# Tongdongq/darwin-gpu

Measured on AMD Instinct MI355X. Metric: GACT GCUPS (DP cells/s) on ~10 kb PacBio-shape reads, higher is better.
Workload: dtype int16x2 (packed); 1 GPU; ecoli10x_self_overlap; tile_size=320, tile_overlap=120, scoring=+1/-1/-1/-1, reads=4642, bases=48503677, candidates=65766, tiles=2185214, parallelism=candidates dealt round-robin over 1 GPU(s), slots_in_flight=4, passes_in_this_process=127, arch=gfx950:sramecc+:xnack-

## Files before the change

darwin-gpu_amd/csrc/gact_lin.hpp:

```cpp
#pragma once

#include "gact_p16s.hpp"

namespace gact {

#ifndef GACT_LIN_MAX3
#define GACT_LIN_MAX3 1
#endif
constexpr int kLinFloor = GACT_LIN_MAX3 ? 1024 : 0;
__host__ __device__ constexpr int lin_base(int g) { return kLinFloor + 40 * (-g) + 8; }
__device__ __forceinline__ uint32_t vconst(uint32_t s)
{
    uint32_t r;
    asm volatile("s_nop 1\n\tv_mov_b32 %0, %1" : "=v"(r) : "s"(s));
    return r;
}

__host__ inline bool p16_lin_ok(int tile, int match, int mismatch, int open, int ext)
{
    const long long steps = (long long)tile + 4 * kGroup + 64 + 48;
    return open == ext && mismatch == ext && ext <= 0 && match >= 0 &&
           p16_tagged_ok(tile, match, mismatch, open, ext) &&
           4 * ((long long)match * (tile + 2) + (long long)(-ext) * steps + kLinFloor) + 3 <= 30000 && match - ext <= 63;
}

#ifndef GACT_LIN_BUILTINS
#define GACT_LIN_BUILTINS 0
#endif
__host__ inline bool lin_col_drift_ok(int match, int ext) { return match - 2 * ext <= 63; }
constexpr bool kLinSplitBuiltins = true;
typedef short LinS2 __attribute__((ext_vector_type(2)));
template <bool BUILTIN = GACT_LIN_BUILTINS>
__device__ __forceinline__ uint32_t lin_max(uint32_t a, uint32_t b)
{
    if constexpr (BUILTIN)
        return __builtin_bit_cast(uint32_t, __builtin_elementwise_max(__builtin_bit_cast(LinS2, a), __builtin_bit_cast(LinS2, b)));
    else
        return pk_max(a, b);
}
__device__ __forceinline__ uint32_t lin_sub(uint32_t a, uint32_t b)
{
#if GACT_LIN_BUILTINS
    return __builtin_bit_cast(uint32_t, (LinS2)(__builtin_bit_cast(LinS2, a) - __builtin_bit_cast(LinS2, b)));
#else
    return pk_sub(a, b);
#endif
}
__device__ __forceinline__ uint32_t pk_mad4v(uint32_t a, uint32_t v_c)
{
    uint32_t r;
    asm("v_pk_mad_u16 %0, %1, 4, %2 op_sel_hi:[1,0,1]" : "=v"(r) : "v"(a), "v"(v_c));
    return r;
}
__device__ __forceinline__ uint32_t pk_max3f(uint32_t a, uint32_t b, uint32_t c)
{
    uint32_t r;
    asm("v_pk_maximum3_f16 %0, %1, %2, %3" : "=v"(r) : "v"(a), "v"(b), "v"(c));
    return r;
}
__device__ __forceinline__ uint32_t pk_max3f_s(uint32_t a, uint32_t s_b, uint32_t c)
{
    uint32_t r;
    asm("v_pk_maximum3_f16 %0, %1, %2, %3" : "=v"(r) : "v"(a), "s"(s_b), "v"(c));
    return r;
}
__device__ __forceinline__ uint32_t pk_max_sgpr(uint32_t a, uint32_t s_b)
{
    uint32_t r;
    asm("v_pk_max_i16 %0, %1, %2" : "=v"(r) : "v"(a), "s"(s_b));
    return r;
}
#define GACT_DPP_SHR1 " row_shr:1 row_mask:0xf bank_mask:0xf"
#define GACT_DPP_ROR1 " row_ror:1 row_mask:0xf bank_mask:0xf"
__device__ __forceinline__ uint32_t lin_hand_shr1(uint32_t h, uint32_t v_k, uint32_t s_old)
{
    uint32_t r;
    asm("v_mov_b32 %0, %3\n\ts_nop 0\n\tv_sub_u32_dpp %0, %1, %2" GACT_DPP_SHR1 : "=&v"(r) : "v"(h), "v"(v_k), "s"(s_old));
    return r;
}
__device__ __forceinline__ uint32_t lin_hand_ror1_shr1(uint32_t h1, uint32_t v_k1, uint32_t h2, uint32_t v_k2)
{
    uint32_t r;
    asm("s_nop 1\n\tv_sub_u32_dpp %0, %1, %2" GACT_DPP_ROR1 "\n\tv_sub_u32_dpp %0, %3, %4" GACT_DPP_SHR1
        : "=&v"(r) : "v"(h1), "v"(v_k1), "v"(h2), "v"(v_k2));
    return r;
}
__device__ __forceinline__ uint32_t lin_hand_scaled_ror1(uint32_t h1, uint32_t v_c)
{
    uint32_t r;
    asm("v_pk_mad_u16 %0, %1, 4, %2 op_sel_hi:[1,0,1]\n\ts_nop 1\n\tv_mov_b32_dpp %0, %0" GACT_DPP_ROR1 : "=&v"(r) : "v"(h1), "v"(v_c));
    return r;
}
__device__ __forceinline__ uint32_t lin_hand_shr1_over(uint32_t first, uint32_t h2, uint32_t v_k2)
{
    asm("s_nop 1\n\tv_sub_u32_dpp %0, %1, %2" GACT_DPP_SHR1 : "+v"(first) : "v"(h2), "v"(v_k2));
    return first;
}
template <bool BUILTIN = GACT_LIN_BUILTINS>
__device__ __forceinline__ uint32_t andn_or(uint32_t a, uint32_t b, uint32_t c)
{
    if constexpr (BUILTIN)
        return __builtin_amdgcn_bitop3_b32(a, b, c, 0xba);
    else {
        uint32_t r;
        asm("v_bitop3_b32 %0, %1, %2, %3 bitop3:0xba" : "=v"(r) : "v"(a), "v"(b), "v"(c));
        return r;
    }
}
__device__ __forceinline__ uint32_t pk_ashr2(uint32_t a)
{
#if GACT_LIN_BUILTINS
    return __builtin_bit_cast(uint32_t, (LinS2)(__builtin_bit_cast(LinS2, a) >> (short)2));
#else
    uint32_t r;
    asm("v_pk_ashrrev_i16 %0, 2, %1 op_sel_hi:[0,1]" : "=v"(r) : "v"(a));
    return r;
#endif
}


__device__ __forceinline__ uint32_t sconst_here(uint32_t lit)
{
    uint32_t r;
    asm volatile("s_mov_b32 %0, %1" : "=s"(r) : "i"(lit));
    return r;
}

template <int CW> struct LinWords {
    static constexpr int kWords = (CW + 1) / 2;
    static constexpr int kUint4 = (kWords + 3) / 4;
};
template <int NW, int LANES, class Fix>
__device__ __forceinline__ void lin_flush(const uint32_t (&acc)[2 * NW], uint4 *qA, uint4 *qB, Fix fix, const bool storeA, const bool storeB)
{
    constexpr int QD = (NW + 3) / 4;
    uint32_t wa[QD * 4], wb[QD * 4];
#pragma unroll
    for (int n = 0; n < QD * 4; n++) {
        wa[n] = n < NW ? fix(__builtin_amdgcn_perm(acc[n < NW ? 2 * n + 1 : 0], acc[n < NW ? 2 * n : 0], 0x05040100u)) : 0u;
        wb[n] = n < NW ? fix(__builtin_amdgcn_perm(acc[n < NW ? 2 * n + 1 : 0], acc[n < NW ? 2 * n : 0], 0x07060302u)) : 0u;
    }
    if (storeA) {
#pragma unroll
        for (int q = 0; q < QD; q++) qA[q * kWsRow] = make_uint4(wa[4 * q], wa[4 * q + 1], wa[4 * q + 2], wa[4 * q + 3]);
    }
    if (storeB) {
#pragma unroll
        for (int q = 0; q < QD; q++) qB[q * kWsRow] = make_uint4(wb[4 * q], wb[4 * q + 1], wb[4 * q + 2], wb[4 * q + 3]);
    }
}

template <int S> struct LinPos { static constexpr int value = S; };
constexpr int kLinTail = -1;
constexpr uint32_t kLinPairSel = 0x06020400u;
constexpr uint32_t kLinPairMask = 0x03030303u;
constexpr uint32_t kLinFlushSelA = 0x05010400u;
constexpr uint32_t kLinFlushSelB = 0x07030602u;
template <int CW>
__device__ __forceinline__ void lin_flush_groups(const uint32_t (&grp)[2 * (CW / 2)], const uint32_t odd, uint4 *qA, uint4 *qB,
                                                 const bool storeA, const bool storeB)
{
    constexpr int NP = CW / 2, NW = LinWords<CW>::kWords, QD = LinWords<CW>::kUint4;
    uint32_t wa[QD * 4], wb[QD * 4];
    const uint32_t sA = sconst_here(kLinFlushSelA), sB = sconst_here(kLinFlushSelB);
#pragma unroll
    for (int n = 0; n < QD * 4; n++) {
        wa[n] = n < NP ? __builtin_amdgcn_perm(grp[n < NP ? 2 * n : 0], grp[n < NP ? 2 * n + 1 : 0], sA)
              : n < NW ? odd & 0xffffu : 0u;
        wb[n] = n < NP ? __builtin_amdgcn_perm(grp[n < NP ? 2 * n : 0], grp[n < NP ? 2 * n + 1 : 0], sB)
              : n < NW ? odd >> 16 : 0u;
    }
    if (storeA) {
#pragma unroll
        for (int q = 0; q < QD; q++) qA[q * kWsRow] = make_uint4(wa[4 * q], wa[4 * q + 1], wa[4 * q + 2], wa[4 * q + 3]);
    }
    if (storeB) {
#pragma unroll
        for (int q = 0; q < QD; q++) qB[q * kWsRow] = make_uint4(wb[4 * q], wb[4 * q + 1], wb[4 * q + 2], wb[4 * q + 3]);
    }
}

constexpr int kLinBandDefault = 48, kLinBandMin = 24, kLinBandQuantum = 1;
struct LinBand {
    int lo[2], hi[2];
    bool full[2];
    __device__ __forceinline__ bool store(int h, int first, int last) const { return full[h] | ((last >= lo[h]) & (first <= hi[h])); }
};
__device__ __forceinline__ void lin_band_range(LinBand &b, int h, int T_end, int behind, int dj_min, int dj_max, int band, bool full)
{
    b.full[h] = full | (band <= 0);
    b.lo[h] = T_end - behind - dj_max - band;
    b.hi[h] = dj_max < 0 ? -0x40000000 : T_end - behind - imax(dj_min, 0) + band;
}

template <int C1, int C2>
__device__ __forceinline__ uint32_t dp_pass_lin_split(const P16Consts &kc, const int gl,
                                                      const uint16_t *__restrict__ ref16,
                                                      const uint32_t (&qb)[C1 + C2],
                                                      const int T_end, const int tB,
                                                      uint32_t *__restrict__ wsA, uint32_t *__restrict__ wsB,
                                                      const int band, const bool fullA, const bool fullB,
                                                      const uint32_t *lut_lds)
{
    constexpr int CT = C1 + C2;
    constexpr int NW = LinWords<C2>::kWords, QD = LinWords<C2>::kUint4;
    constexpr int LAG = kGroup;
    const int g = (int)(int16_t)(kc.ext & 0xffffu);
    const uint32_t gv = vconst(kc.next), g4v = vconst(kc.next4), c3v = vconst(kc.c3), onev = vconst(kc.one),
                   dtv = vconst(kc.next4 + kc.tag1),
                   c2v = vconst(kc.tag2);
    const uint32_t psel = sconst_here(kLinPairSel);
    uint32_t Z1 = pk2(lin_base(g) + gl * g), Z2 = pk2(lin_base(g) + (gl + LAG) * g);
    uint32_t G[CT];
    uint32_t acc[2 * NW];
    uint32_t grp[2 * (C2 / 2)], odd = 0;
#pragma unroll
    for (int c = 0; c < CT; c++) G[c] = c < C1 ? Z1 : Z2;
#pragma unroll
    for (int c = 0; c < 2 * NW; c++) acc[c] = 0;
    uint32_t H1 = Z1, H2 = Z2;
    uint32_t Hdiag1 = Z1, Hdiag2 = Z2;

    typedef __attribute__((address_space(3))) const uint8_t LdsByte;
    typedef __attribute__((address_space(3))) const uint32_t LdsWord;
    LdsByte *const lut_plain = (LdsByte *)lut_lds, *const lut_tagged = (LdsByte *)(lut_lds + 1);
    auto row = [](LdsByte *table, uint32_t stream_byte) { return *(LdsWord *)(table + stream_byte); };
    LdsByte *rp = (LdsByte *)(ref16 + (1 - LAG));
    uint32_t rb1 = row(lut_plain, rp[2 * LAG]), rb1b = row(lut_plain, rp[2 * LAG + 1]);
    uint32_t rb2 = row(lut_plain, rp[0]), rb2b = row(lut_plain, rp[1]);
    rp += 2;

#define GACT_SB() __builtin_amdgcn_sched_barrier(0)
    uint32_t sb1 = 0, sb1b = 0, sb2 = 0, sb2b = 0;
    auto ask_bytes = [&](const bool r1, const bool r2) {
        if (r2) { sb2 = rp[0]; sb2b = rp[1]; }
        if (r1) { sb1 = rp[2 * LAG]; sb1b = rp[2 * LAG + 1]; }
        rp += 2;
    };
    auto ask_rows = [&](const bool r1, const bool r2, const bool tag2) {
        if (r1) { rb1 = row(lut_plain, sb1); rb1b = row(lut_plain, sb1b); }
        if (r2) { rb2 = row(tag2 ? lut_tagged : lut_plain, sb2); rb2b = row(tag2 ? lut_tagged : lut_plain, sb2b); }
    };
    auto upper_all = [&](uint32_t (&U)[CT], const bool tag2, const uint32_t Zr2) {
        uint32_t P[CT];
#pragma unroll
        for (int c = 0; c < CT; c++) P[c] = __builtin_amdgcn_perm(c < C1 ? rb1b : rb2b, c < C1 ? rb1 : rb2, qb[c]);
        GACT_SB();
#pragma unroll
        for (int c = 0; c < CT; c++) U[c] = (c == 0 ? Hdiag1 : c == C1 ? Hdiag2 : G[c - 1]) + P[c];
        ask_rows(true, true, tag2);
        GACT_SB();
        if (GACT_LIN_MAX3) {
#pragma unroll
            for (int c = 0; c < CT; c++)
                U[c] = pk_max3f(U[c], c < C1 ? Z1 : Zr2, G[c]);
        } else {
#pragma unroll
            for (int c = 0; c < CT; c++) U[c] = lin_max(U[c], c < C1 ? Z1 : Zr2);
            GACT_SB();
#pragma unroll
            for (int c = 0; c < CT; c++) U[c] = lin_max(U[c], G[c]);
        }
        GACT_SB();
    };

    auto step = [&]() {
        ask_bytes(true, true);
        Z1 += gv; Z2 += gv;
        const uint32_t Hl1 = (uint32_t)dpp_row_shr1((int)H1, (int)Z1);
        const uint32_t Hl2 = (uint32_t)dpp_row_shr1((int)H2, dpp_row_ror1((int)H1));
        uint32_t U[CT];
        upper_all(U, false, Z2);
        Hdiag1 = Hl1; Hdiag2 = Hl2;
        uint32_t Ha = Hl1, Hb = Hl2;
        static_assert(C2 >= C1, "region 2 is the longer chain");
#pragma unroll
        for (int c = 0; c < C1; c++) {
            const uint32_t Da = Ha - gv, Db = Hb - gv;
            GACT_SB();
            G[c] = lin_max(U[c], Da); G[C1 + c] = lin_max(U[C1 + c], Db);
            GACT_SB();
            Ha = G[c]; Hb = G[C1 + c];
        }
#pragma unroll
        for (int c = 2 * C1; c < CT; c++) { G[c] = lin_max(U[c], Hb - gv); Hb = G[c]; }
        H1 = Ha; H2 = Hb;
    };
    auto step_r1 = [&]() {
        ask_bytes(true, false);
        Z1 += gv; Z2 += gv;
        const uint32_t Hl1 = (uint32_t)dpp_row_shr1((int)H1, (int)Z1);
        uint32_t P[C1], U[C1];
#pragma unroll
        for (int c = 0; c < C1; c++) P[c] = __builtin_amdgcn_perm(rb1b, rb1, qb[c]);
        GACT_SB();
#pragma unroll
        for (int c = 0; c < C1; c++) U[c] = (c == 0 ? Hdiag1 : G[c - 1]) + P[c];
        ask_rows(true, false, false);
        GACT_SB();
#pragma unroll
        for (int c = 0; c < C1; c++) U[c] = GACT_LIN_MAX3 ? pk_max3f(U[c], Z1, G[c]) : lin_max(lin_max(U[c], Z1), G[c]);
        GACT_SB();
        Hdiag1 = Hl1;
        uint32_t Ha = Hl1;
#pragma unroll
        for (int c = 0; c < C1; c++) { G[c] = lin_max(U[c], Ha - gv); Ha = G[c]; }
        H1 = Ha;
    };

    uint32_t Z24 = 0;
    static_assert(C2 >= 3 && (C2 & 1), "the last pair is filed while the unpaired slot is computed");
    auto file_group = [&](const int S, const int c, const uint32_t x) {
        uint32_t &r = grp[c - 2 + (S >> 2)];
        r = (S & 3) ? pk_shl_add4(r, x) : x;
    };
    auto step_tagged = [&](auto pos) {
        constexpr int S = decltype(pos)::value;
        constexpr bool blk = S != kLinTail;
        ask_bytes(true, true);
        Z1 += gv; Z24 += g4v;
        const uint32_t Hl1 = (uint32_t)dpp_row_shr1((int)H1, (int)Z1);
        const uint32_t Hl2 = (uint32_t)dpp_row_shr1((int)H2, dpp_row_ror1((int)pk_mad4v(H1, c2v)));
        uint32_t U[CT];
        upper_all(U, true, Z24);
        Hdiag1 = Hl1; Hdiag2 = Hl2;
        uint32_t Ha = Hl1, Hb = Hl2;
        uint32_t tprev = 0, Hq = 0, x = 0;
#pragma unroll
        for (int c = 0; c < C2; c++) {
            const bool both = c < C1;
            const bool filed = blk && c >= 2 && !(c & 1);
            uint32_t Da = 0;
            const uint32_t Db = Hb - dtv;
            if (both) Da = Ha - gv;
            if (filed) x &= kLinPairMask;
            GACT_SB();
            const uint32_t Hp = lin_max(U[C1 + c], Db);
            if (both) { G[c] = lin_max(U[c], Da); Ha = G[c]; }
            if (!blk && c > 0) acc[c - 1] = pk_shl_add4(acc[c - 1], tprev);
            if (filed) file_group(S, c, x);
            GACT_SB();
            G[C1 + c] = andn_or(Hp, c3v, c2v);
            if (!blk || c == C2 - 1) tprev = Hp & c3v;
            else if (c & 1) x = __builtin_amdgcn_perm(Hp, Hq, psel);
            else Hq = Hp;
            GACT_SB();
            Hb = G[C1 + c];
        }
        if (!blk) acc[C2 - 1] = pk_shl_add4(acc[C2 - 1], tprev);
        else odd = S ? pk_shl_add4(odd, tprev) : tprev;
        H1 = Ha; H2 = Hb;
    };
    auto step_tagged_r2 = [&](auto pos) {
        constexpr int S = decltype(pos)::value;
        constexpr bool blk = S != kLinTail;
        ask_bytes(false, true);
        Z24 += g4v;
        const uint32_t Hl2 = (uint32_t)dpp_row_shr1((int)H2, dpp_row_ror1((int)pk_mad4v(H1, c2v)));
        uint32_t P[C2], U[C2];
#pragma unroll
        for (int c = 0; c < C2; c++) P[c] = __builtin_amdgcn_perm(rb2b, rb2, qb[C1 + c]);
        GACT_SB();
#pragma unroll
        for (int c = 0; c < C2; c++) U[c] = (c == 0 ? Hdiag2 : G[C1 + c - 1]) + P[c];
        ask_rows(false, true, true);
        GACT_SB();
#pragma unroll
        for (int c = 0; c < C2; c++) U[c] = GACT_LIN_MAX3 ? pk_max3f(U[c], Z24, G[C1 + c]) : lin_max(lin_max(U[c], Z24), G[C1 + c]);
        GACT_SB();
        Hdiag2 = Hl2;
        uint32_t Hb = Hl2;
        uint32_t tprev = 0, Hq = 0, x = 0;
#pragma unroll
        for (int c = 0; c < C2; c++) {
            const bool filed = blk && c >= 2 && !(c & 1);
            const uint32_t Db = Hb - dtv;
            if (filed) x &= kLinPairMask;
            GACT_SB();
            const uint32_t Hp = lin_max(U[c], Db);
            if (!blk && c > 0) acc[c - 1] = pk_shl_add4(acc[c - 1], tprev);
            if (filed) file_group(S, c, x);
            GACT_SB();
            G[C1 + c] = andn_or(Hp, c3v, c2v);
            if (!blk || c == C2 - 1) tprev = Hp & c3v;
            else if (c & 1) x = __builtin_amdgcn_perm(Hp, Hq, psel);
            else Hq = Hp;
            GACT_SB();
            Hb = G[C1 + c];
        }
        if (!blk) acc[C2 - 1] = pk_shl_add4(acc[C2 - 1], tprev);
        else odd = S ? pk_shl_add4(odd, tprev) : tprev;
        H2 = Hb;
    };
#define GACT_LIN_BLOCK8(f) do { f(LinPos<0>{}); f(LinPos<1>{}); f(LinPos<2>{}); f(LinPos<3>{}); \
                                f(LinPos<4>{}); f(LinPos<5>{}); f(LinPos<6>{}); f(LinPos<7>{}); } while (0)
#undef GACT_SB
    auto enter_tagged = [&]() {
#pragma unroll
        for (int c = C1; c < CT; c++) G[c] = pk_mad4v(G[c], c2v);
        H2 = pk_mad4v(H2, c2v);
        Hdiag2 = pk_mad4v(Hdiag2, c2v);
        Z24 = pk_mad4v(Z2, c3v);
        rb2 = row(lut_tagged, rp[-2]); rb2b = row(lut_tagged, rp[-1]);
    };

    int t = 1;
    for (const int tP = imin(LAG, imin(tB - 1, T_end)); t <= tP; t++) step_r1();
    if (t > 1) {
#pragma unroll
        for (int c = C1; c < CT; c++) G[c] = Z2;
        H2 = Z2; Hdiag2 = Z2;
        rb2 = row(lut_plain, rp[-2]); rb2b = row(lut_plain, rp[-1]);
    }
    const int tU = imin(tB - 1, T_end);
    for (; t + 1 <= tU; t += 2) { step(); step(); }
    if (t <= tU) { step(); t++; }
    const bool tagged = t <= T_end;
    if (tagged) enter_tagged();
    uint4 *qA = reinterpret_cast<uint4 *>(wsA) + gl;
    uint4 *qB = reinterpret_cast<uint4 *>(wsB) + gl;
    LinBand bd;
    {
        const int q1 = (band >> 16) - 1, b = band & 0xffff;
        const int u_lo = kGroup - 1 - (gl & ~q1), u_hi = kGroup - 1 - (gl | q1);
        LinBand lo_, hi_;
        lin_band_range(lo_, 0, T_end, u_lo, C2 * u_lo, C2 * u_lo + C2 - 1, b, fullA);
        lin_band_range(hi_, 0, T_end, u_hi, C2 * u_hi, C2 * u_hi + C2 - 1, b, fullA);
        bd.lo[0] = bd.lo[1] = lo_.lo[0]; bd.hi[0] = bd.hi[1] = hi_.hi[0];
        bd.full[0] = fullA | (b <= 0); bd.full[1] = fullB | (b <= 0);
    }
    int k = 0;
    while (t + 7 <= T_end && t <= T_end - LAG) {
        GACT_LIN_BLOCK8(step_tagged);
        t += 8; k += 8;
        lin_flush_groups<C2>(grp, odd, qA, qB, bd.store(0, t - 8, t - 1), bd.store(1, t - 8, t - 1));
        qA += QD * kWsRow;
        qB += QD * kWsRow;
    }
    while (t + 7 <= T_end) {
        GACT_LIN_BLOCK8(step_tagged_r2);
        t += 8; k += 8;
        lin_flush_groups<C2>(grp, odd, qA, qB, bd.store(0, t - 8, t - 1), bd.store(1, t - 8, t - 1));
        qA += QD * kWsRow;
        qB += QD * kWsRow;
    }
#undef GACT_LIN_BLOCK8
    for (; t <= T_end - LAG; t++, k++) step_tagged(LinPos<kLinTail>{});
    for (; t <= T_end; t++, k++) step_tagged_r2(LinPos<kLinTail>{});
    if (k & 7) {
        const int sh = 2 * (8 - (k & 7));
        lin_flush<NW, kGroup>(acc, qA, qB, [sh](uint32_t w) { return ((w & 0xffffu) << sh & 0xffffu) | ((w >> 16) << sh << 16); },
                              bd.store(0, t - (k & 7), t - 1), bd.store(1, t - (k & 7), t - 1));
    }
    return tagged ? pk_ashr2(lin_sub(H2 | kc.c3, Z24)) : lin_sub(H2, Z2);
}

template <int C1, int C2>
__device__ __forceinline__ uint32_t dp_pass_lin_split_col(const P16Consts &kc, const int gl,
                                                      const uint16_t *__restrict__ ref16,
                                                      const uint32_t (&qb)[C1 + C2],
                                                      const int T_end, const int tB,
                                                      uint32_t *__restrict__ wsA, uint32_t *__restrict__ wsB,
                                                      const int band, const bool fullA, const bool fullB,
                                                      const uint32_t *lut_lds)
{
    constexpr int CT = C1 + C2;
    constexpr int NW = LinWords<C2>::kWords, QD = LinWords<C2>::kUint4;
    constexpr int LAG = kGroup;
    const int g = (int)(int16_t)(kc.ext & 0xffffu);
    const uint32_t gs = kc.next, g4s = kc.next4;
    const uint32_t k1v = vconst((uint32_t)(C1 - 1) * kc.next),
                   k2v = vconst((uint32_t)(C2 - 1) * kc.next);
    uint32_t c3v = 0, onev = 0, c2v = 0,
             k24v = 0,
             k12v = 0;
    const uint32_t psel = sconst_here(kLinPairSel);
    constexpr int NWIN = C2 + 1;
    uint32_t W[NWIN], T[C2];
#pragma unroll
    for (int k = 0; k < NWIN; k++) W[k] = pk2(lin_base(g) + (k - 1) * (-g));
#pragma unroll
    for (int c = 0; c < C2; c++) T[c] = 0;
    auto bump = [](uint32_t &z, const uint32_t by) { asm("s_add_u32 %0, %0, %1" : "+s"(z) : "s"(by) : "scc"); };
    auto advance = [&](const int nW, const bool tagged_too) {
#pragma unroll
        for (int k = 0; k < NWIN; k++) if (k < nW) { if (tagged_too) bump(W[k], gs); else W[k] += gs; }
        if (tagged_too) {
#pragma unroll
            for (int c = 0; c < C2; c++) bump(T[c], g4s);
        }
    };
    uint32_t G[CT];
    uint32_t acc[2 * NW];
    uint32_t grp[2 * (C2 / 2)], odd = 0;
#pragma unroll
    for (int c = 0; c < CT; c++) G[c] = W[(c < C1 ? c : c - C1) + 1];
#pragma unroll
    for (int c = 0; c < 2 * NW; c++) acc[c] = 0;
    uint32_t H1 = W[C1], H2 = W[C2];
    uint32_t Hdiag1 = W[0], Hdiag2 = W[0];

    typedef __attribute__((address_space(3))) const uint8_t LdsByte;
    typedef __attribute__((address_space(3))) const uint32_t LdsWord;
    LdsByte *const lut_plain = (LdsByte *)lut_lds, *const lut_tagged = (LdsByte *)(lut_lds + 1);
    auto row = [](LdsByte *table, uint32_t stream_byte) { return *(LdsWord *)(table + stream_byte); };
    LdsByte *rp = (LdsByte *)(ref16 + (1 - LAG));
    uint32_t rb1 = row(lut_plain, rp[2 * LAG]), rb1b = row(lut_plain, rp[2 * LAG + 1]);
    uint32_t rb2 = row(lut_plain, rp[0]), rb2b = row(lut_plain, rp[1]);
    rp += 2;

#define GACT_SB() __builtin_amdgcn_sched_barrier(0)
    uint32_t sb1 = 0, sb1b = 0, sb2 = 0, sb2b = 0;
    auto ask_bytes = [&](const bool r1, const bool r2) {
        if (r2) { sb2 = rp[0]; sb2b = rp[1]; }
        if (r1) { sb1 = rp[2 * LAG]; sb1b = rp[2 * LAG + 1]; }
        rp += 2;
    };
    auto ask_rows = [&](const bool r1, const bool r2, const bool tag2) {
        if (r1) { rb1 = row(lut_plain, sb1); rb1b = row(lut_plain, sb1b); }
        if (r2) { rb2 = row(tag2 ? lut_tagged : lut_plain, sb2); rb2b = row(tag2 ? lut_tagged : lut_plain, sb2b); }
    };
    auto upper_all = [&](uint32_t (&U)[CT], const bool tag2) {
        uint32_t P[CT];
#pragma unroll
        for (int c = 0; c < CT; c++) P[c] = __builtin_amdgcn_perm(c < C1 ? rb1b : rb2b, c < C1 ? rb1 : rb2, qb[c]);
        GACT_SB();
#pragma unroll
        for (int c = 0; c < CT; c++) U[c] = (c == 0 ? Hdiag1 : c == C1 ? Hdiag2 : G[c - 1]) + P[c];
        ask_rows(true, true, tag2);
        GACT_SB();
        if (GACT_LIN_MAX3) {
#pragma unroll
            for (int c = 0; c < CT; c++)
                U[c] = pk_max3f_s(U[c], c < C1 ? W[c + 1] : tag2 ? T[c - C1] : W[c - C1 + 1], G[c]);
        } else {
#pragma unroll
            for (int c = 0; c < CT; c++) U[c] = pk_max_sgpr(U[c], c < C1 ? W[c + 1] : tag2 ? T[c - C1] : W[c - C1 + 1]);
            GACT_SB();
#pragma unroll
            for (int c = 0; c < CT; c++) U[c] = lin_max<kLinSplitBuiltins>(U[c], G[c]);
        }
        GACT_SB();
    };

    auto step = [&]() {
        ask_bytes(true, true);
        advance(NWIN, false);
        const uint32_t Hl1 = lin_hand_shr1(H1, k1v, W[0]);
        const uint32_t Hl2 = lin_hand_ror1_shr1(H1, k1v, H2, k2v);
        uint32_t U[CT];
        upper_all(U, false);
        Hdiag1 = Hl1; Hdiag2 = Hl2;
        uint32_t Ha = Hl1, Hb = Hl2;
        static_assert(C2 >= C1, "region 2 is the longer chain");
#pragma unroll
        for (int c = 0; c < C1; c++) {
            G[c] = lin_max<kLinSplitBuiltins>(U[c], Ha); G[C1 + c] = lin_max<kLinSplitBuiltins>(U[C1 + c], Hb);
            GACT_SB();
            Ha = G[c]; Hb = G[C1 + c];
        }
#pragma unroll
        for (int c = 2 * C1; c < CT; c++) { G[c] = lin_max<kLinSplitBuiltins>(U[c], Hb); Hb = G[c]; }
        H1 = Ha; H2 = Hb;
    };
    auto step_r1 = [&]() {
        ask_bytes(true, false);
        advance(C1 + 1, false);
        const uint32_t Hl1 = lin_hand_shr1(H1, k1v, W[0]);
        uint32_t P[C1], U[C1];
#pragma unroll
        for (int c = 0; c < C1; c++) P[c] = __builtin_amdgcn_perm(rb1b, rb1, qb[c]);
        GACT_SB();
#pragma unroll
        for (int c = 0; c < C1; c++) U[c] = (c == 0 ? Hdiag1 : G[c - 1]) + P[c];
        ask_rows(true, false, false);
        GACT_SB();
#pragma unroll
        for (int c = 0; c < C1; c++) U[c] = GACT_LIN_MAX3 ? pk_max3f_s(U[c], W[c + 1], G[c]) : lin_max<kLinSplitBuiltins>(pk_max_sgpr(U[c], W[c + 1]), G[c]);
        GACT_SB();
        Hdiag1 = Hl1;
        uint32_t Ha = Hl1;
#pragma unroll
        for (int c = 0; c < C1; c++) { G[c] = lin_max<kLinSplitBuiltins>(U[c], Ha); Ha = G[c]; }
        H1 = Ha;
    };

    static_assert(C2 >= 3 && (C2 & 1), "the last pair is filed while the unpaired slot is computed");
    auto file_group = [&](const int S, const int c, const uint32_t x) {
        uint32_t &r = grp[c - 2 + (S >> 2)];
        r = (S & 3) ? pk_shl_add4(r, x) : x;
    };
    auto step_tagged = [&](auto pos) {
        constexpr int S = decltype(pos)::value;
        constexpr bool blk = S != kLinTail;
        ask_bytes(true, true);
        advance(C1 + 1, true);
        const uint32_t Hl1 = lin_hand_shr1(H1, k1v, W[0]);
        const uint32_t Hl2 = lin_hand_shr1_over(lin_hand_scaled_ror1(H1, k12v), H2, k24v);
        uint32_t U[CT];
        upper_all(U, true);
        Hdiag1 = Hl1; Hdiag2 = Hl2;
        uint32_t Ha = Hl1, Hb = Hl2;
        uint32_t tprev = 0, Hq = 0, x = 0;
#pragma unroll
        for (int c = 0; c < C2; c++) {
            const bool both = c < C1;
            const bool filed = blk && c >= 2 && !(c & 1);
            const uint32_t Db = Hb - onev;
            if (filed) x &= kLinPairMask;
            GACT_SB();
            const uint32_t Hp = lin_max<kLinSplitBuiltins>(U[C1 + c], Db);
            if (both) { G[c] = lin_max<kLinSplitBuiltins>(U[c], Ha); Ha = G[c]; }
            if (!blk && c > 0) acc[c - 1] = pk_shl_add4(acc[c - 1], tprev);
            if (filed) file_group(S, c, x);
            GACT_SB();
            G[C1 + c] = andn_or<kLinSplitBuiltins>(Hp, c3v, c2v);
            if (!blk || c == C2 - 1) tprev = Hp & c3v;
            else if (c & 1) x = __builtin_amdgcn_perm(Hp, Hq, psel);
            else Hq = Hp;
            GACT_SB();
            Hb = G[C1 + c];
        }
        if (!blk) acc[C2 - 1] = pk_shl_add4(acc[C2 - 1], tprev);
        else odd = S ? pk_shl_add4(odd, tprev) : tprev;
        H1 = Ha; H2 = Hb;
    };
    auto step_tagged_r2 = [&](auto pos) {
        constexpr int S = decltype(pos)::value;
        constexpr bool blk = S != kLinTail;
        ask_bytes(false, true);
        advance(0, true);
        const uint32_t Hl2 = lin_hand_shr1_over(lin_hand_scaled_ror1(H1, k12v), H2, k24v);
        uint32_t P[C2], U[C2];
#pragma unroll
        for (int c = 0; c < C2; c++) P[c] = __builtin_amdgcn_perm(rb2b, rb2, qb[C1 + c]);
        GACT_SB();
#pragma unroll
        for (int c = 0; c < C2; c++) U[c] = (c == 0 ? Hdiag2 : G[C1 + c - 1]) + P[c];
        ask_rows(false, true, true);
        GACT_SB();
#pragma unroll
        for (int c = 0; c < C2; c++) U[c] = GACT_LIN_MAX3 ? pk_max3f_s(U[c], T[c], G[C1 + c]) : lin_max<kLinSplitBuiltins>(pk_max_sgpr(U[c], T[c]), G[C1 + c]);
        GACT_SB();
        Hdiag2 = Hl2;
        uint32_t Hb = Hl2;
        uint32_t tprev = 0, Hq = 0, x = 0;
#pragma unroll
        for (int c = 0; c < C2; c++) {
            const bool filed = blk && c >= 2 && !(c & 1);
            const uint32_t Db = Hb - onev;
            if (filed) x &= kLinPairMask;
            GACT_SB();
            const uint32_t Hp = lin_max<kLinSplitBuiltins>(U[c], Db);
            if (!blk && c > 0) acc[c - 1] = pk_shl_add4(acc[c - 1], tprev);
            if (filed) file_group(S, c, x);
            GACT_SB();
            G[C1 + c] = andn_or<kLinSplitBuiltins>(Hp, c3v, c2v);
            if (!blk || c == C2 - 1) tprev = Hp & c3v;
            else if (c & 1) x = __builtin_amdgcn_perm(Hp, Hq, psel);
            else Hq = Hp;
            GACT_SB();
            Hb = G[C1 + c];
        }
        if (!blk) acc[C2 - 1] = pk_shl_add4(acc[C2 - 1], tprev);
        else odd = S ? pk_shl_add4(odd, tprev) : tprev;
        H2 = Hb;
    };
#define GACT_LIN_BLOCK8(f) do { f(LinPos<0>{}); f(LinPos<1>{}); f(LinPos<2>{}); f(LinPos<3>{}); \
                                f(LinPos<4>{}); f(LinPos<5>{}); f(LinPos<6>{}); f(LinPos<7>{}); } while (0)
#undef GACT_SB
    auto enter_tagged = [&]() {
        c3v = vconst(kc.c3); onev = vconst(kc.one); c2v = vconst(kc.tag2);
        k24v = vconst((uint32_t)(C2 - 1) * kc.next4);
        k12v = vconst(pk2(2 + 4 * (C1 - 1) * g));
#pragma unroll
        for (int c = C1; c < CT; c++) G[c] = pk_mad4v(G[c], c2v);
        H2 = pk_mad4v(H2, c2v);
        Hdiag2 = pk_mad4v(Hdiag2, c2v);
#pragma unroll
        for (int c = 0; c < C2; c++) T[c] = (W[c + 1] << 2) + kc.c3;
        rb2 = row(lut_tagged, rp[-2]); rb2b = row(lut_tagged, rp[-1]);
    };

    int t = 1;
    for (const int tP = imin(LAG, imin(tB - 1, T_end)); t <= tP; t++) step_r1();
    if (t > 1) {
#pragma unroll
        for (int k = C1 + 1; k < NWIN; k++) W[k] = W[k - 1] + gs;
#pragma unroll
        for (int c = C1; c < CT; c++) G[c] = W[c - C1 + 1];
        H2 = W[C2]; Hdiag2 = W[0];
        rb2 = row(lut_plain, rp[-2]); rb2b = row(lut_plain, rp[-1]);
    }
    const int tU = imin(tB - 1, T_end);
    for (; t + 1 <= tU; t += 2) { step(); step(); }
    if (t <= tU) { step(); t++; }
    const bool tagged = t <= T_end;
    if (tagged) enter_tagged();
    uint4 *qA = reinterpret_cast<uint4 *>(wsA) + gl;
    uint4 *qB = reinterpret_cast<uint4 *>(wsB) + gl;
    LinBand bd;
    {
        const int q1 = (band >> 16) - 1, b = band & 0xffff;
        const int u_lo = kGroup - 1 - (gl & ~q1), u_hi = kGroup - 1 - (gl | q1);
        LinBand lo_, hi_;
        lin_band_range(lo_, 0, T_end, u_lo, C2 * u_lo, C2 * u_lo + C2 - 1, b, fullA);
        lin_band_range(hi_, 0, T_end, u_hi, C2 * u_hi, C2 * u_hi + C2 - 1, b, fullA);
        bd.lo[0] = bd.lo[1] = lo_.lo[0]; bd.hi[0] = bd.hi[1] = hi_.hi[0];
        bd.full[0] = fullA | (b <= 0); bd.full[1] = fullB | (b <= 0);
    }
    int k = 0;
    while (t + 7 <= T_end && t <= T_end - LAG) {
        GACT_LIN_BLOCK8(step_tagged);
        t += 8; k += 8;
        lin_flush_groups<C2>(grp, odd, qA, qB, bd.store(0, t - 8, t - 1), bd.store(1, t - 8, t - 1));
        qA += QD * kWsRow;
        qB += QD * kWsRow;
    }
    while (t + 7 <= T_end) {
        GACT_LIN_BLOCK8(step_tagged_r2);
        t += 8; k += 8;
        lin_flush_groups<C2>(grp, odd, qA, qB, bd.store(0, t - 8, t - 1), bd.store(1, t - 8, t - 1));
        qA += QD * kWsRow;
        qB += QD * kWsRow;
    }
#undef GACT_LIN_BLOCK8
    for (; t <= T_end - LAG; t++, k++) step_tagged(LinPos<kLinTail>{});
    for (; t <= T_end; t++, k++) step_tagged_r2(LinPos<kLinTail>{});
    if (k & 7) {
        const int sh = 2 * (8 - (k & 7));
        lin_flush<NW, kGroup>(acc, qA, qB, [sh](uint32_t w) { return ((w & 0xffffu) << sh & 0xffffu) | ((w >> 16) << sh << 16); },
                              bd.store(0, t - (k & 7), t - 1), bd.store(1, t - (k & 7), t - 1));
    }
    return tagged ? pk_ashr2(lin_sub(H2 | kc.c3, T[C2 - 1])) : lin_sub(H2, W[C2]);
}
#undef GACT_DPP_SHR1
#undef GACT_DPP_ROR1

template <int C, int LANES, bool AMAX>
__device__ __forceinline__ uint32_t dp_pass_lin(const P16Consts &kc, const int gl,
                                                const uint16_t *__restrict__ ref16,
                                                const uint32_t (&qb)[C],
                                                const int T_end, const int tB,
                                                uint32_t *__restrict__ wsA, uint32_t *__restrict__ wsB,
                                                const int cqA, const int cqB, const int (*RQ)[2], P16Best *pb,
                                                const int col_from, const int band, const int QA, const int QB,
                                                const bool fullA, const bool fullB)
{
    constexpr int NW = LinWords<C>::kWords, QD = LinWords<C>::kUint4;
    const bool store = AMAX || gl * C + C >= col_from;
    LinBand bd;
    {
        const int q1 = AMAX ? 0 : (band >> 16) - 1, b = AMAX ? 0 : band & 0xffff;
        const int g_lo = gl & ~q1, g_hi = gl | q1;
        LinBand lo_, hi_;
        lin_band_range(lo_, 0, T_end, (imax(QA, 1) - 1) / C - g_lo, QA - g_lo * C - C, QA - g_lo * C - 1, b, fullA);
        lin_band_range(lo_, 1, T_end, (imax(QB, 1) - 1) / C - g_lo, QB - g_lo * C - C, QB - g_lo * C - 1, b, fullB);
        lin_band_range(hi_, 0, T_end, (imax(QA, 1) - 1) / C - g_hi, QA - g_hi * C - C, QA - g_hi * C - 1, b, fullA);
        lin_band_range(hi_, 1, T_end, (imax(QB, 1) - 1) / C - g_hi, QB - g_hi * C - C, QB - g_hi * C - 1, b, fullB);
        bd = lo_;
        bd.hi[0] = hi_.hi[0] < 0 ? (lo_.hi[0] < 0 ? lo_.hi[0] : T_end) : hi_.hi[0];
        bd.hi[1] = hi_.hi[1] < 0 ? (lo_.hi[1] < 0 ? lo_.hi[1] : T_end) : hi_.hi[1];
    }
    static_assert(!AMAX || LANES == kGroup, "first tiles run on the 16-lane layout");
    const int g = (int)(int16_t)(kc.ext & 0xffffu);
    const uint32_t gv = vconst(kc.next), g4v = vconst(kc.next4), c3v = vconst(kc.c3), onev = vconst(kc.one),
                   dtv = vconst(kc.next4 + kc.tag1),
                   c2v = vconst(kc.tag2), lut1v = vconst(0x01010101u);
    uint32_t Z = pk2(lin_base(g) + gl * g);
    uint32_t G[C];
    uint32_t acc[2 * NW];
#pragma unroll
    for (int c = 0; c < C; c++) G[c] = Z;
#pragma unroll
    for (int c = 0; c < 2 * NW; c++) acc[c] = 0;
    uint32_t G_last = Z, Hdiag = Z;

    uint32_t bk[AMAX ? C : 1];
    int lane_best[2] = {-1, -1};
    uint32_t col_x0 = 0;
    int t_first = 0, rows[2] = {0, 0};
    if (AMAX) {
#pragma unroll
        for (int c = 0; c < C; c++) bk[c] = 0xffffffffu;
        const int ncA = imin(imax(RQ[0][1] - gl * C, 0), C), ncB = imin(imax(RQ[1][1] - gl * C, 0), C);
        col_x0 = ((uint32_t)(-ncA) & 0xffffu) | ((uint32_t)(-ncB) << 16);
        t_first = gl + 1;
        rows[0] = RQ[0][0]; rows[1] = RQ[1][0];
    }

    auto lut = [&](uint32_t amount) { return kc.dsub >> (amount & 31u); };
    auto lut4 = [&](uint32_t amount) { return kc.dsub4 >> (amount & 31u); };
    uint32_t lutA = 0, lutB = 0;
    { const uint32_t w = ref16[1]; lutA = lut(w & 0xffu); lutB = lut(w >> 8); }

    auto shr1 = [](uint32_t v, uint32_t old) {
        return (uint32_t)(LANES == 32 ? dpp_shr1_32((int)v, (int)old) : dpp_row_shr1((int)v, (int)old));
    };

#define GACT_SB() __builtin_amdgcn_sched_barrier(0)
    auto upper_all = [&](uint32_t (&U)[C], const bool tag2, const uint32_t Zr) {
        uint32_t P[C];
#pragma unroll
        for (int c = 0; c < C; c++) P[c] = __builtin_amdgcn_perm(lutB, lutA, qb[c]);
        GACT_SB();
#pragma unroll
        for (int c = 0; c < C; c++) U[c] = (c == 0 ? Hdiag : G[c - 1]) + P[c];
        (void)tag2;
        GACT_SB();
        if (GACT_LIN_MAX3) {
#pragma unroll
            for (int c = 0; c < C; c++) U[c] = pk_max3f(U[c], Zr, G[c]);
        } else {
#pragma unroll
            for (int c = 0; c < C; c++) U[c] = lin_max(U[c], Zr);
            GACT_SB();
#pragma unroll
            for (int c = 0; c < C; c++) U[c] = lin_max(U[c], G[c]);
        }
        GACT_SB();
    };

    auto step = [&](const int t) {
        const uint32_t w_next = ref16[t + 1];
        Z += gv;
        const uint32_t Hl0 = shr1(G_last, Z);
        uint32_t U[C];
        upper_all(U, false, Z);
        Hdiag = Hl0;
        uint32_t Hl = Hl0;
#pragma unroll
        for (int c = 0; c < C; c++) { G[c] = lin_max(U[c], Hl - gv); Hl = G[c]; }
        G_last = Hl;
        lutA = lut(w_next & 0xffu); lutB = lut(w_next >> 8);
    };

    uint32_t Z4 = 0, Z8 = 0;
    auto step_tagged = [&](const int t) {
        const uint32_t w_next = ref16[t + 1];
        Z4 += g4v;
        uint32_t key_c = 0;
        if (AMAX) {
            Z8 += g4v + g4v;
            const uint32_t sidx = (uint32_t)(t - tB) & 7u, row0 = (uint32_t)(t - t_first);
            const uint32_t ka = row0 < (uint32_t)rows[0] ? sidx : ((uint32_t)kKeyBias & 0xffffu);
            const uint32_t kb = row0 < (uint32_t)rows[1] ? sidx : ((uint32_t)kKeyBias & 0xffffu);
            key_c = lin_sub(ka | (kb << 16), Z8);
        }
        const uint32_t Hl0 = shr1(G_last, Z4 - onev);
        uint32_t U[C];
        upper_all(U, true, Z4);
        Hdiag = Hl0;
        uint32_t Hl = Hl0, tprev = 0;
#pragma unroll
        for (int c = 0; c < C; c++) {
            const uint32_t Db = Hl - dtv;
            GACT_SB();
            const uint32_t Hp = lin_max(U[c], Db);
            if (c > 0) {
                acc[c - 1] = pk_shl_add4(acc[c - 1], tprev);
                if (AMAX) bk[c - 1] = lin_max(bk[c - 1], pk_mad_vvv(G[c - 1], kc.tag2, key_c));
            }
            GACT_SB();
            G[c] = andn_or(Hp, c3v, c2v);
            tprev = Hp & c3v;
            GACT_SB();
            Hl = G[c];
        }
        acc[C - 1] = pk_shl_add4(acc[C - 1], tprev);
        if (AMAX) bk[C - 1] = lin_max(bk[C - 1], pk_mad_vvv(G[C - 1], kc.tag2, key_c));
        G_last = Hl;
        lutA = lut4(w_next & 0xffu) + lut1v; lutB = lut4(w_next >> 8) + lut1v;
    };
#undef GACT_SB
    auto enter_tagged = [&]() {
#pragma unroll
        for (int c = 0; c < C; c++) G[c] = pk_mad4v(G[c], c2v);
        G_last = pk_mad4v(G_last, c2v);
        Hdiag = pk_mad4v(Hdiag, c2v);
        Z4 = pk_mad4v(Z, c3v);
        Z8 = Z4 + Z4 - c2v;
        lutA = (lutA << 2) + lut1v; lutB = (lutB << 2) + lut1v;
    };

    auto fold = [&](const int kblk) {
        uint32_t m = 0xffffffffu, rel = 0, x = col_x0;
#pragma unroll
        for (int c = 0; c < C; c++) {
            const uint32_t v = pk_sign(x);
            x = pk_add(x, kc.one);
            const uint32_t key = pk_mad_m1(v, pk_add(bk[AMAX ? c : 0], kc.one));
            const uint32_t keep = pk_sign(lin_sub(key, m));
            rel = pk_mad_m1(keep, rel);
            m = lin_max(m, key);
            bk[AMAX ? c : 0] = 0xffffffffu;
        }
#pragma unroll
        for (int h = 0; h < 2; h++) {
            const int m16 = (int)(m << (16 - 16 * h)) >> 16;
            const int col = ((int)(rel << (16 - 16 * h)) >> 16) + C;
            const int rec = ((m16 >> 3) << 15) | ((kblk + (m16 & 7)) << 5) | col;
            lane_best[h] = imax(lane_best[h], m16 < 0 ? -1 : rec);
        }
    };

    int t = 1;
    for (; t < tB && t <= T_end; t++) step(t);
    const bool tagged = t <= T_end;
    if (tagged) enter_tagged();
    uint4 *qA = reinterpret_cast<uint4 *>(wsA) + gl;
    uint4 *qB = reinterpret_cast<uint4 *>(wsB) + gl;
    int k = 0;
    while (t + 7 <= T_end) {
        for (int s8 = 0; s8 < 8; s8++, t++) step_tagged(t);
        k += 8;
        lin_flush<NW, LANES>(acc, qA, qB, [](uint32_t w) { return w; }, store && bd.store(0, t - 8, t - 1), store && bd.store(1, t - 8, t - 1));
        qA += QD * kWsRow;
        qB += QD * kWsRow;
        if (AMAX) fold(k - 8);
    }
    for (; t <= T_end; t++, k++) step_tagged(t);
    if (AMAX) {
        if (k & 7) fold(k & ~7);
#pragma unroll
        for (int h = 0; h < 2; h++) {
            const int rec = lane_best[h];
            int best = 0, bi = 0, bj = 0;
            if (rec >= 0) {
                best = rec >> 15;
                bi = tB + ((rec >> 5) & 1023) - gl;
                bj = gl * C + (rec & 31) + 1;
            }
#pragma unroll
            for (int mm = 1; mm < kGroup; mm <<= 1) {
                const int ob = __shfl_xor(best, mm, kGroup);
                const int oi = __shfl_xor(bi, mm, kGroup);
                const int oj = __shfl_xor(bj, mm, kGroup);
                const bool take = (ob > best) | ((ob == best) & ((oi > bi) | ((oi == bi) & (oj > bj))));
                best = take ? ob : best;
                bi = take ? oi : bi;
                bj = take ? oj : bj;
            }
            pb->best[h] = best; pb->bi[h] = bi; pb->bj[h] = bj;
        }
    }
    if (k & 7) {
        const int sh = 2 * (8 - (k & 7));
        lin_flush<NW, LANES>(acc, qA, qB, [sh](uint32_t w) { return ((w & 0xffffu) << sh & 0xffffu) | ((w >> 16) << sh << 16); },
                             store && bd.store(0, t - (k & 7), t - 1), store && bd.store(1, t - (k & 7), t - 1));
    }
    if (AMAX) return 0;
    uint32_t ga = G[0], gb = G[0];
#pragma unroll
    for (int c = 1; c < C; c++) { ga = (c == cqA) ? G[c] : ga; gb = (c == cqB) ? G[c] : gb; }
    const uint32_t pick = __builtin_amdgcn_perm(gb, ga, 0x07060100u);
    return tagged ? pk_ashr2(lin_sub(pick | kc.c3, Z4)) : lin_sub(pick, Z);
}

struct WideLayoutLin : UniformLayout<10, 32, true> {
    static constexpr int kWalkFmt = 3, kWalkQuads = LinWords<10>::kUint4;
#ifndef GACT_WALK_SPAN
#define GACT_WALK_SPAN 16
#endif
    static constexpr int kWalkSpan = GACT_WALK_SPAN;
#ifndef GACT_WIDE_LIN_BLOCKS
#define GACT_WIDE_LIN_BLOCKS 3
#endif
    static constexpr int kBlocksPerCu = GACT_WIDE_LIN_BLOCKS;
    static constexpr bool kEndAligned = true;
    template <bool RAW>
    __device__ static uint32_t pass(const P16Consts &kc, int gl, const uint16_t *ref16, const uint32_t (&qb)[10], int T_end,
                                    int tB, uint32_t *wsA, uint32_t *wsB, const PairTile &pt)
    {
        static_assert(!RAW, "the linear-gap pass reads 2-bit sets");
        return dp_pass_lin<10, 32, false>(kc, gl, ref16, qb, T_end, tB, wsA, wsB, (imax(pt.Q[0], 1) - 1) % 10,
                                          (imax(pt.Q[1], 1) - 1) % 10, nullptr, nullptr, pt.col_from, pt.band, pt.Q[0], pt.Q[1],
                                          pt.full[0], pt.full[1]);
    }
    __device__ static int fin_lane(int Q) { return (imax(Q, 1) - 1) / 10; }
};

#ifndef GACT_LIN_BLOCKS_PER_CU
#define GACT_LIN_BLOCKS_PER_CU 3
#endif
template <int C1, int C2> struct SplitLayoutLin : SplitLayout<C1, C2, true> {
    static constexpr int kBlocksPerCu = GACT_LIN_BLOCKS_PER_CU;
    static constexpr int kWalkFmt = 3, kWalkQuads = LinWords<C2>::kUint4;
    static constexpr int kWalkSpan = GACT_WALK_SPAN;
    static constexpr bool kEndAligned = true;
    static constexpr int kLutWords = kLinLutWords;
    static constexpr bool kColDrift = true;
    using Base = SplitLayout<C1, C2, true>;
    template <bool RAW>
    __device__ static void load(const SeqSetDev &rs, const SeqSetDev &qf, const SeqSetDev &qr,
                                const PairTile &pt, int gl, uint8_t *ref8, uint8_t *q8, uint32_t (&qb)[C1 + C2], uint32_t *stage)
    {
        static_assert(!RAW, "the linear-gap pass reads 2-bit sets");
        load_pair_packed<C1 + C2, kGroup, typename Base::Cols, true, kLinPadRow>(rs, qf, qr, pt, gl, ref8, Base::G::kRefBytes, Base::G::kRow0, q8,
                                                                                 Base::G::kTileMax, qb, stage, typename Base::Cols{});
    }
    template <bool RAW>
    __device__ static uint32_t pass(const P16Consts &kc, int gl, const uint16_t *ref16, const uint32_t (&qb)[C1 + C2],
                                    int T_end, int tB, uint32_t *wsA, uint32_t *wsB, const PairTile &pt)
    {
        static_assert(!RAW, "the linear-gap pass reads 2-bit sets");
        return dp_pass_lin_split_col<C1, C2>(kc, gl, ref16, qb, T_end, tB, wsA, wsB, pt.band, pt.full[0], pt.full[1], pt.lut);
    }
    __device__ static int fin_lane(int Q) { (void)Q; return kGroup - 1; }
};

template <int C1, int C2> struct SplitLayoutLinRow : SplitLayoutLin<C1, C2> {
    static constexpr bool kColDrift = false;
    template <bool RAW>
    __device__ static uint32_t pass(const P16Consts &kc, int gl, const uint16_t *ref16, const uint32_t (&qb)[C1 + C2],
                                    int T_end, int tB, uint32_t *wsA, uint32_t *wsB, const PairTile &pt)
    {
        static_assert(!RAW, "the linear-gap pass reads 2-bit sets");
        return dp_pass_lin_split<C1, C2>(kc, gl, ref16, qb, T_end, tB, wsA, wsB, pt.band, pt.full[0], pt.full[1], pt.lut);
    }
};

template <int C1, int C2> struct SplitLayoutLinRowTeam : SplitLayoutLinRow<C1, C2> {
    static constexpr bool kTeamWalk = true;
};

template <int C1, int C2> struct SplitLayoutLinTeam : SplitLayoutLin<C1, C2> {
    static constexpr bool kTeamWalk = true;
};

}
```

Before: 9363 GCUPS.

## Slide precomputed boundary-offset strips instead of bumping scalars every step

The per-step scalar advance of the boundary arrays W and T is replaced inside 8-step blocks by precomputed strips that hold each step's offsets in extra SGPRs. Each step indexes the strip at its block position, and the whole strip is bumped once per block with batched s_add instructions. This removes the per-step SALU adds from the inner DP loop. In exchange it uses about 7 more SGPRs per array, which could affect register pressure or occupancy, and it relies on the tail loops restoring the original offsets correctly.

```diff
diff --git a/darwin-gpu_amd/csrc/gact_lin.hpp b/darwin-gpu_amd/csrc/gact_lin.hpp
--- a/darwin-gpu_amd/csrc/gact_lin.hpp
+++ b/darwin-gpu_amd/csrc/gact_lin.hpp
@@ -455,6 +455,37 @@
     return tagged ? pk_ashr2(lin_sub(H2 | kc.c3, Z24)) : lin_sub(H2, Z2);
 }
 
+#ifndef GACT_LIN_SLIDE
+#define GACT_LIN_SLIDE 1
+#endif
+constexpr int kLinBlock = 8;
+__host__ __device__ constexpr int lin_strip_len(int n, int steps = kLinBlock) { return GACT_LIN_SLIDE ? n + steps - 1 : n; }
+__host__ __device__ constexpr int lin_strip_at(int S, int k) { return GACT_LIN_SLIDE && S != kLinTail ? S + k : k; }
+template <int N, int STEPS = kLinBlock, int LEN>
+__host__ __device__ __forceinline__ void lin_strip_enter(uint32_t (&s)[LEN], const uint32_t by)
+{
+    static_assert(lin_strip_len(N, STEPS) <= LEN, "the strip fits its registers");
+#pragma unroll
+    for (int k = 0; k < N; k++) s[k] += by;
+#pragma unroll
+    for (int k = N; k < lin_strip_len(N, STEPS); k++) s[k] = s[k - 1] + by;
+}
+template <int N, int LEN>
+__host__ __device__ __forceinline__ void lin_strip_leave(uint32_t (&s)[LEN], const uint32_t by)
+{
+#pragma unroll
+    for (int k = 0; k < N; k++) s[k] -= by;
+}
+template <int N, int STEPS = kLinBlock, int LEN, class Add4, class Add1>
+__host__ __device__ __forceinline__ void lin_strip_slide(uint32_t (&s)[LEN], const uint32_t by_block, Add4 add4, Add1 add1)
+{
+    constexpr int M = lin_strip_len(N, STEPS);
+#pragma unroll
+    for (int j = 0; j + 4 <= M; j += 4) add4(s[j], s[j + 1], s[j + 2], s[j + 3], by_block);
+#pragma unroll
+    for (int j = M & ~3; j < M; j++) add1(s[j], by_block);
+}
+
 template <int C1, int C2>
 __device__ __forceinline__ uint32_t dp_pass_lin_split_col(const P16Consts &kc, const int gl,
                                                       const uint16_t *__restrict__ ref16,
@@ -476,11 +507,13 @@
              k12v = 0;
     const uint32_t psel = sconst_here(kLinPairSel);
     constexpr int NWIN = C2 + 1;
-    uint32_t W[NWIN], T[C2];
+    uint32_t W[lin_strip_len(NWIN)], T[lin_strip_len(C2)];
 #pragma unroll
     for (int k = 0; k < NWIN; k++) W[k] = pk2(lin_base(g) + (k - 1) * (-g));
 #pragma unroll
-    for (int c = 0; c < C2; c++) T[c] = 0;
+    for (int c = 0; c < lin_strip_len(C2); c++) T[c] = 0;
+#pragma unroll
+    for (int k = NWIN; k < lin_strip_len(NWIN); k++) W[k] = 0;
     auto bump = [](uint32_t &z, const uint32_t by) { asm("s_add_u32 %0, %0, %1" : "+s"(z) : "s"(by) : "scc"); };
     auto advance = [&](const int nW, const bool tagged_too) {
 #pragma unroll
@@ -489,6 +522,10 @@
 #pragma unroll
             for (int c = 0; c < C2; c++) bump(T[c], g4s);
         }
+    };
+    auto bump4 = [](uint32_t &z0, uint32_t &z1, uint32_t &z2, uint32_t &z3, const uint32_t by) {
+        asm("s_add_u32 %0, %0, %4\n\ts_add_u32 %1, %1, %4\n\ts_add_u32 %2, %2, %4\n\ts_add_u32 %3, %3, %4"
+            : "+s"(z0), "+s"(z1), "+s"(z2), "+s"(z3) : "s"(by) : "scc");
     };
     uint32_t G[CT];
     uint32_t acc[2 * NW];
@@ -520,7 +557,7 @@
         if (r1) { rb1 = row(lut_plain, sb1); rb1b = row(lut_plain, sb1b); }
         if (r2) { rb2 = row(tag2 ? lut_tagged : lut_plain, sb2); rb2b = row(tag2 ? lut_tagged : lut_plain, sb2b); }
     };
-    auto upper_all = [&](uint32_t (&U)[CT], const bool tag2) {
+    auto upper_all = [&](uint32_t (&U)[CT], const bool tag2, const int o) {
         uint32_t P[CT];
 #pragma unroll
         for (int c = 0; c < CT; c++) P[c] = __builtin_amdgcn_perm(c < C1 ? rb1b : rb2b, c < C1 ? rb1 : rb2, qb[c]);
@@ -532,10 +569,10 @@
         if (GACT_LIN_MAX3) {
 #pragma unroll
             for (int c = 0; c < CT; c++)
-                U[c] = pk_max3f_s(U[c], c < C1 ? W[c + 1] : tag2 ? T[c - C1] : W[c - C1 + 1], G[c]);
+                U[c] = pk_max3f_s(U[c], c < C1 ? W[o + c + 1] : tag2 ? T[o + c - C1] : W[o + c - C1 + 1], G[c]);
         } else {
 #pragma unroll
-            for (int c = 0; c < CT; c++) U[c] = pk_max_sgpr(U[c], c < C1 ? W[c + 1] : tag2 ? T[c - C1] : W[c - C1 + 1]);
+            for (int c = 0; c < CT; c++) U[c] = pk_max_sgpr(U[c], c < C1 ? W[o + c + 1] : tag2 ? T[o + c - C1] : W[o + c - C1 + 1]);
             GACT_SB();
 #pragma unroll
             for (int c = 0; c < CT; c++) U[c] = lin_max<kLinSplitBuiltins>(U[c], G[c]);
@@ -543,13 +580,14 @@
         GACT_SB();
     };
 
-    auto step = [&]() {
+    auto step = [&](auto pos) {
+        constexpr int S = decltype(pos)::value, o = lin_strip_at(S, 0);
         ask_bytes(true, true);
-        advance(NWIN, false);
-        const uint32_t Hl1 = lin_hand_shr1(H1, k1v, W[0]);
+        if (!GACT_LIN_SLIDE || S == kLinTail) advance(NWIN, false);
+        const uint32_t Hl1 = lin_hand_shr1(H1, k1v, W[o]);
         const uint32_t Hl2 = lin_hand_ror1_shr1(H1, k1v, H2, k2v);
         uint32_t U[CT];
-        upper_all(U, false);
+        upper_all(U, false, o);
         Hdiag1 = Hl1; Hdiag2 = Hl2;
         uint32_t Ha = Hl1, Hb = Hl2;
         static_assert(C2 >= C1, "region 2 is the longer chain");
@@ -593,12 +631,13 @@
     auto step_tagged = [&](auto pos) {
         constexpr int S = decltype(pos)::value;
         constexpr bool blk = S != kLinTail;
+        constexpr int o = lin_strip_at(S, 0);
         ask_bytes(true, true);
-        advance(C1 + 1, true);
-        const uint32_t Hl1 = lin_hand_shr1(H1, k1v, W[0]);
+        if (!GACT_LIN_SLIDE || !blk) advance(C1 + 1, true);
+        const uint32_t Hl1 = lin_hand_shr1(H1, k1v, W[o]);
         const uint32_t Hl2 = lin_hand_shr1_over(lin_hand_scaled_ror1(H1, k12v), H2, k24v);
         uint32_t U[CT];
-        upper_all(U, true);
+        upper_all(U, true, o);
         Hdiag1 = Hl1; Hdiag2 = Hl2;
         uint32_t Ha = Hl1, Hb = Hl2;
         uint32_t tprev = 0, Hq = 0, x = 0;
@@ -628,8 +667,9 @@
     auto step_tagged_r2 = [&](auto pos) {
         constexpr int S = decltype(pos)::value;
         constexpr bool blk = S != kLinTail;
+        constexpr int o = lin_strip_at(S, 0);
         ask_bytes(false, true);
-        advance(0, true);
+        if (!GACT_LIN_SLIDE || !blk) advance(0, true);
         const uint32_t Hl2 = lin_hand_shr1_over(lin_hand_scaled_ror1(H1, k12v), H2, k24v);
         uint32_t P[C2], U[C2];
 #pragma unroll
@@ -640,7 +680,7 @@
         ask_rows(false, true, true);
         GACT_SB();
 #pragma unroll
-        for (int c = 0; c < C2; c++) U[c] = GACT_LIN_MAX3 ? pk_max3f_s(U[c], T[c], G[C1 + c]) : lin_max<kLinSplitBuiltins>(pk_max_sgpr(U[c], T[c]), G[C1 + c]);
+        for (int c = 0; c < C2; c++) U[c] = GACT_LIN_MAX3 ? pk_max3f_s(U[c], T[o + c], G[C1 + c]) : lin_max<kLinSplitBuiltins>(pk_max_sgpr(U[c], T[o + c]), G[C1 + c]);
         GACT_SB();
         Hdiag2 = Hl2;
         uint32_t Hb = Hl2;
@@ -693,8 +733,16 @@
         rb2 = row(lut_plain, rp[-2]); rb2b = row(lut_plain, rp[-1]);
     }
     const int tU = imin(tB - 1, T_end);
-    for (; t + 1 <= tU; t += 2) { step(); step(); }
-    if (t <= tU) { step(); t++; }
+#if GACT_LIN_SLIDE
+    lin_strip_enter<NWIN>(W, gs);
+    for (; t + kLinBlock - 1 <= tU; t += kLinBlock) {
+        GACT_LIN_BLOCK8(step);
+        lin_strip_slide<NWIN>(W, gs * kLinBlock, bump4, bump);
+    }
+    lin_strip_leave<NWIN>(W, gs);
+#endif
+    for (; t + 1 <= tU; t += 2) { step(LinPos<kLinTail>{}); step(LinPos<kLinTail>{}); }
+    if (t <= tU) { step(LinPos<kLinTail>{}); t++; }
     const bool tagged = t <= T_end;
     if (tagged) enter_tagged();
     uint4 *qA = reinterpret_cast<uint4 *>(wsA) + gl;
@@ -710,9 +758,16 @@
         bd.full[0] = fullA | (b <= 0); bd.full[1] = fullB | (b <= 0);
     }
     int k = 0;
+#if GACT_LIN_SLIDE
+    if (tagged) { lin_strip_enter<C1 + 1>(W, gs); lin_strip_enter<C2>(T, g4s); }
+#endif
     while (t + 7 <= T_end && t <= T_end - LAG) {
         GACT_LIN_BLOCK8(step_tagged);
         t += 8; k += 8;
+#if GACT_LIN_SLIDE
+        lin_strip_slide<C1 + 1>(W, gs * kLinBlock, bump4, bump);
+        lin_strip_slide<C2>(T, g4s * kLinBlock, bump4, bump);
+#endif
         lin_flush_groups<C2>(grp, odd, qA, qB, bd.store(0, t - 8, t - 1), bd.store(1, t - 8, t - 1));
         qA += QD * kWsRow;
         qB += QD * kWsRow;
@@ -720,11 +775,17 @@
     while (t + 7 <= T_end) {
         GACT_LIN_BLOCK8(step_tagged_r2);
         t += 8; k += 8;
+#if GACT_LIN_SLIDE
+        lin_strip_slide<C2>(T, g4s * kLinBlock, bump4, bump);
+#endif
         lin_flush_groups<C2>(grp, odd, qA, qB, bd.store(0, t - 8, t - 1), bd.store(1, t - 8, t - 1));
         qA += QD * kWsRow;
         qB += QD * kWsRow;
     }
 #undef GACT_LIN_BLOCK8
+#if GACT_LIN_SLIDE
+    if (tagged) { lin_strip_leave<C1 + 1>(W, gs); lin_strip_leave<C2>(T, g4s); }
+#endif
     for (; t <= T_end - LAG; t++, k++) step_tagged(LinPos<kLinTail>{});
     for (; t <= T_end; t++, k++) step_tagged_r2(LinPos<kLinTail>{});
     if (k & 7) {
```

After: 9629 GCUPS (median of 6 runs). 2.8% higher.
